# UoB-HPC/stdpar-nbody

Hardware: AMD Instinct MI355X
Metric: body-steps/sec + %FP64 peak, 3D double all-pairs N=2^20 at 1/2/4/8 GPUs (higher is better)
Workload: dtype f64

## Files before the change

### stdpar-nbody_amd/csrc/all_pairs.hip

```cpp
#include "common.hpp"

#include <atomic>
#include <cstdlib>
#include <mutex>
#include <type_traits>
#include <vector>

namespace nbody {

constexpr int kBlock = 256;
constexpr int kWaves = kBlock / 64;

struct ap_config {
  int split = 0;
  int tpt   = 0;
  int path  = 0;
};
static std::atomic<uint32_t> g_ap_default{0};

static ap_config ap_config_of(const nbody_state* s) {
  const uint32_t t = s->tuning ? s->tuning : g_ap_default.load(std::memory_order_relaxed);
  ap_config c;
  c.split = int(t & 15u);
  c.tpt   = int((t >> 4) & 3u);
  c.path  = int((t >> 6) & 3u);
  return c;
}

template <typename T, int D, int R, int JS>
__global__ __launch_bounds__(kBlock) void all_pairs_force_kernel(const T* __restrict__ m, const T* __restrict__ x,
                                                                 T* __restrict__ a, T c, uint32_t sz, uint32_t first,
                                                                 uint32_t count, const k1_rule* __restrict__ rule) {
  [[maybe_unused]] constexpr T e2 = T(0);
#define K1_SOFT false
#include "k1_tile_body.inc"
#undef K1_SOFT
}
template <typename T, int D, int R, int JS>
__global__ __launch_bounds__(kBlock) void all_pairs_softened_kernel(const T* __restrict__ m, const T* __restrict__ x,
                                                                    T* __restrict__ a, T c, uint32_t sz, uint32_t first,
                                                                    uint32_t count, T e2) {
  const k1_rule* const rule = nullptr;
#define K1_SOFT true
#include "k1_tile_body.inc"
#undef K1_SOFT
}

template <typename T, int D>
__global__ __launch_bounds__(kBlock) void pack_sources_kernel(const T* __restrict__ m, const T* __restrict__ x,
                                                              src_rec<T, D>* __restrict__ out, uint32_t sz, uint32_t padded) {
  const uint32_t j = blockIdx.x * kBlock + threadIdx.x;
  if (j >= padded) return;
  src_rec<T, D> r;
#pragma unroll
  for (int k = 0; k < 3; ++k) r.p[k] = (k < D && j < sz) ? x[uint64_t(j) * D + (k < D ? k : 0)] : T(0);
  r.m    = j < sz ? m[j] : T(0);
  out[j] = r;
}

template <typename T>
struct k1_prepare_tail {
  uint32_t turn_words;
};
template <>
struct k1_prepare_tail<double> {
  uint32_t turn_words;
  uint32_t bpc;
  double* cbox;
  double* pbox;
};
template <typename T, int D, bool PACK, bool MOMENTS>
__global__ __launch_bounds__(kBlock) void k1_prepare_kernel(const T* __restrict__ m, const T* __restrict__ x, src_rec<T, D>* __restrict__ out,
                                                            cst_batch* __restrict__ cst, uint32_t sz, uint32_t padded, k1_rule* rule, double* partial,
                                                            uint32_t* turn, k1_prepare_tail<T> tail) {
  constexpr bool BOX        = PACK && MOMENTS && sizeof(T) == 8;
  const uint32_t turn_words = tail.turn_words;
  [[maybe_unused]] uint32_t bpc = 0;
  [[maybe_unused]] T *cbox = nullptr, *pbox = nullptr;
  if constexpr (BOX) bpc = tail.bpc, cbox = tail.cbox, pbox = tail.pbox;
  const uint32_t j = blockIdx.x * kBlock + threadIdx.x;
  T p[D];
#pragma unroll
  for (int k = 0; k < D; ++k) p[k] = j < sz ? x[uint64_t(j) * D + k] : T(0);
  if constexpr (PACK) {
    if (j < padded) {
      src_rec<T, D> r;
#pragma unroll
      for (int k = 0; k < 3; ++k) r.p[k] = k < D ? p[k < D ? k : 0] : T(0);
      r.m    = j < sz ? m[j] : T(0);
      out[j] = r;
      if constexpr (sizeof(T) == 8) {
        const src_cst<T> k  = src_cst<T>::of(r.m);
        cst[j / 2].m15[j % 2]   = k.m15;
        cst[j / 2].m1875[j % 2] = k.m1875;
      }
    }
  }
  __shared__ double red[2 * D][kWaves];
  __shared__ T bred[BOX ? 2 * D : 1][kWaves];
  __shared__ bool last_s;
  const int lane = threadIdx.x & 63, wave = threadIdx.x >> 6;
  if constexpr (MOMENTS) {
    double s1[D], s2[D];
#pragma unroll
    for (int k = 0; k < D; ++k) {
      const double d = j < sz ? double(p[k]) - double(x[k]) : 0.0;
      s1[k] = d;
      s2[k] = d * d;
    }
#pragma unroll
    for (int k = 0; k < D; ++k)
      for (int off = 32; off > 0; off >>= 1) {
        s1[k] += __shfl_xor(s1[k], off, 64);
        s2[k] += __shfl_xor(s2[k], off, 64);
      }
    if (lane == 0) {
#pragma unroll
      for (int k = 0; k < D; ++k) {
        red[k][wave]     = s1[k];
        red[D + k][wave] = s2[k];
      }
    }
    if constexpr (BOX) {
      if (bpc != 0) {
        bool finite = true;
#pragma unroll
        for (int k = 0; k < D; ++k) finite = finite && (p[k] - p[k]) == T(0);
        T lo[D], hi[D];
#pragma unroll
        for (int k = 0; k < D; ++k) {
          lo[k] = finite ? p[k] : -T(__builtin_inf());
          hi[k] = finite ? p[k] : T(__builtin_inf());
        }
#pragma unroll
        for (int k = 0; k < D; ++k)
          for (int off = 32; off > 0; off >>= 1) {
            lo[k] = __builtin_fmin(lo[k], __shfl_xor(lo[k], off, 64));
            hi[k] = __builtin_fmax(hi[k], __shfl_xor(hi[k], off, 64));
          }
        if (lane == 0) {
#pragma unroll
          for (int k = 0; k < D; ++k) {
            bred[k][wave]     = lo[k];
            bred[D + k][wave] = hi[k];
          }
        }
      }
    }
    __syncthreads();
    if (threadIdx.x < 2 * D) {
      double v = red[threadIdx.x][0];
      for (int w = 1; w < kWaves; ++w) v += red[threadIdx.x][w];
      __hip_atomic_store(partial + size_t(blockIdx.x) * (2 * D) + threadIdx.x, v, __ATOMIC_RELAXED, __HIP_MEMORY_SCOPE_AGENT);
    }
    if constexpr (BOX) {
      if (bpc != 0 && threadIdx.x >= 64 && threadIdx.x < 64 + 2 * D) {
        const int q = int(threadIdx.x) - 64;
        T v         = bred[q][0];
        for (int w = 1; w < kWaves; ++w) v = q < D ? __builtin_fmin(v, bred[q][w]) : __builtin_fmax(v, bred[q][w]);
        __hip_atomic_store(pbox + size_t(blockIdx.x) * (2 * D) + q, v, __ATOMIC_RELAXED, __HIP_MEMORY_SCOPE_AGENT);
      }
    }
  }
  __builtin_amdgcn_s_waitcnt(0);
  __syncthreads();
  if (threadIdx.x == 0) last_s = __hip_atomic_fetch_add(&rule->ticket, 1u, __ATOMIC_RELAXED, __HIP_MEMORY_SCOPE_AGENT) == gridDim.x - 1u;
  __syncthreads();
  if (!last_s) return;
  if constexpr (MOMENTS) {
    double acc = 0.0;
    constexpr int G = kBlock / (2 * D), U = 8;
    const int q = threadIdx.x % (2 * D), g = threadIdx.x / (2 * D);
    if (g < G) {
      for (uint32_t b0 = uint32_t(g); b0 < gridDim.x; b0 += G * U) {
        double v[U];
#pragma unroll
        for (int u = 0; u < U; ++u) {
          const uint32_t b = b0 + uint32_t(u) * G;
          v[u] = b < gridDim.x ? __hip_atomic_load(partial + size_t(b) * (2 * D) + q, __ATOMIC_RELAXED, __HIP_MEMORY_SCOPE_AGENT) : 0.0;
        }
#pragma unroll
        for (int u = 0; u < U; ++u) acc += v[u];
      }
    }
    __shared__ double fin[kBlock];
    fin[threadIdx.x] = g < G ? acc : 0.0;
    __syncthreads();
    if (threadIdx.x < 2 * D) {
      double tot = 0.0;
#pragma unroll 6
      for (int gg = 0; gg < G; ++gg) tot += fin[gg * (2 * D) + threadIdx.x];
      fin[threadIdx.x] = tot;
    }
    __syncthreads();
    if (threadIdx.x == 0) {
      double vol = 1.0;
#pragma unroll
      for (int k = 0; k < D; ++k) {
        const double mean = fin[k] / double(sz), var = fin[D + k] / double(sz) - mean * mean;
        vol *= var > 0.0 ? __builtin_sqrt(12.0 * var) : 0.0;
      }
      rule->volume = vol;
      rule->sparse = vol >= kFarMinVolume<D> ? 1u : 0u;
    }
  }
  if constexpr (BOX) {
    if (bpc != 0) {
      const uint32_t nchunks = (gridDim.x + bpc - 1) / bpc;
      const uint32_t sub     = threadIdx.x & 15u;
      for (uint32_t c0 = 0; c0 < nchunks; c0 += kBlock / 16) {
        const uint32_t c  = c0 + (threadIdx.x >> 4);
        const uint32_t b1 = c < nchunks ? min(gridDim.x, (c + 1u) * bpc) : 0u;
        T lo[D], hi[D];
#pragma unroll
        for (int k = 0; k < D; ++k) lo[k] = T(__builtin_inf()), hi[k] = -T(__builtin_inf());
        for (uint32_t b0 = c * bpc + sub; b0 < b1; b0 += 16u * 4u) {
          T v[4][2 * D];
#pragma unroll
          for (int u = 0; u < 4; ++u) {
            const uint32_t b = b0 + 16u * uint32_t(u);
#pragma unroll
            for (int q = 0; q < 2 * D; ++q)
              v[u][q] = b < b1 ? __hip_atomic_load(pbox + size_t(b) * (2 * D) + q, __ATOMIC_RELAXED, __HIP_MEMORY_SCOPE_AGENT)
                               : (q < D ? T(__builtin_inf()) : -T(__builtin_inf()));
          }
#pragma unroll
          for (int u = 0; u < 4; ++u)
#pragma unroll
            for (int k = 0; k < D; ++k) {
              lo[k] = __builtin_fmin(lo[k], v[u][k]);
              hi[k] = __builtin_fmax(hi[k], v[u][D + k]);
            }
        }
#pragma unroll
        for (int k = 0; k < D; ++k)
          for (int off = 8; off > 0; off >>= 1) {
            lo[k] = __builtin_fmin(lo[k], __shfl_xor(lo[k], off, 64));
            hi[k] = __builtin_fmax(hi[k], __shfl_xor(hi[k], off, 64));
          }
        if (c < nchunks && sub == 0) {
#pragma unroll
          for (int k = 0; k < D; ++k) {
            cbox[size_t(c) * (2 * D) + k]     = lo[k];
            cbox[size_t(c) * (2 * D) + D + k] = hi[k];
          }
        }
      }
    }
  }
  for (uint32_t w = threadIdx.x; w < turn_words; w += kBlock) turn[w] = 0u;
  if (threadIdx.x == 0) __hip_atomic_store(&rule->ticket, 0u, __ATOMIC_RELAXED, __HIP_MEMORY_SCOPE_AGENT);
}

template <int JS>
constexpr int kSgprWaves = JS > kWaves ? JS : kWaves;

constexpr uint32_t kTurnSpins  = 1u << 26;
constexpr uint32_t kTurnPoison = 0xffffffffu;
struct k1_status {
  uint32_t err, block, group, chunk;
  unsigned long long polls, waits;
};
struct k1_handoff {
  void* sums;
  uint32_t* turn;
  k1_status* status;
  uint32_t spins;
  uint32_t delay;
  uint32_t late;
};
constexpr size_t kBoxHeaderBytes = 64;
template <typename T>
struct k1_rule_arg {
  const k1_rule* rule;
};
template <>
struct k1_rule_arg<double> {
  const k1_rule* rule;
  const double* box;
};
template <typename T, int D, int R, int JS, int RULE = 0>
__global__ __launch_bounds__(64 * kSgprWaves<JS>) void all_pairs_force_sgpr_kernel(const src_rec<T, D>* __restrict__ packed,
                                                                                   const cst_batch* __restrict__ cst,
                                                                                   const T* __restrict__ x, T* a, T c, uint32_t sz,
                                                                                   uint32_t first, uint32_t count,
                                                                                   uint32_t tiles_per_chunk, k1_handoff h,
                                                                                   k1_rule_arg<T> ra) {
  [[maybe_unused]] constexpr T e2 = T(0);
  const k1_rule* __restrict__ const rule = ra.rule;
  [[maybe_unused]] const T* __restrict__ box = nullptr;
  if constexpr (sizeof(T) == 8) box = ra.box;
#define K1_SOFT false
#include "k1_sgpr_body.inc"
#undef K1_SOFT
}
template <typename T, int D, int R, int JS>
__global__ __launch_bounds__(64 * kSgprWaves<JS>) void all_pairs_softened_sgpr_kernel(const src_rec<T, D>* __restrict__ packed,
                                                                                      const cst_batch* __restrict__ cst,
                                                                                      const T* __restrict__ x, T* a, T c, uint32_t sz,
                                                                                      uint32_t first, uint32_t count,
                                                                                      uint32_t tiles_per_chunk, k1_handoff h, T e2) {
  constexpr int RULE = 0;
  const k1_rule* const rule = nullptr;
  [[maybe_unused]] const T* const box = nullptr;
#define K1_SOFT true
#include "k1_sgpr_body.inc"
#undef K1_SOFT
}

namespace {
struct scratch_buf {
  void* ptr  = nullptr;
  size_t cap = 0;
};
struct packed_slot {
  int device;
  hipStream_t stream;
  scratch_buf buf[8];
  std::vector<void*> retired;
  bool k1_dirty  = false;
  bool k1_failed = false;
};
std::mutex g_packed_mu;
std::vector<packed_slot> g_packed_slots;
}

int ap_scratch_get(hipStream_t st, int which, size_t bytes, void** out) {
  const int dev = stream_device(st);
  std::lock_guard<std::mutex> lock(g_packed_mu);
  packed_slot* slot = nullptr;
  for (auto& sl : g_packed_slots)
    if (sl.stream == st && sl.device == dev) slot = &sl;
  if (slot && slot->buf[which].cap >= bytes) {
    *out = slot->buf[which].ptr;
    return NBODY_OK;
  }
  hipStreamCaptureStatus cs = hipStreamCaptureStatusNone;
  if (st != nullptr) (void)hipStreamIsCapturing(st, &cs);
  if (cs != hipStreamCaptureStatusNone) {
    set_error("all-pairs: the scratch buffers of this stream must exist before a step is recorded "
              "(call nbody_all_pairs_force once outside nbody_graph_begin/end, or use a context from nbody_create)");
    return NBODY_ERR_STATE;
  }
  if (!slot) {
    g_packed_slots.push_back({dev, st, {}, {}});
    slot = &g_packed_slots.back();
  }
  void* fresh = nullptr;
  NB_HIP(hipMalloc(&fresh, bytes));
  if (which == 4 || which == 3 || which == 7) {
    if (hipError_t e = hipMemsetAsync(fresh, 0, bytes, st); e != hipSuccess) {
      (void)hipFree(fresh);
      return hip_fail(e, "hipMemsetAsync(K1 scratch)", __FILE__, __LINE__);
    }
  }
  if (slot->buf[which].ptr) slot->retired.push_back(slot->buf[which].ptr);
  slot->buf[which].ptr = fresh;
  slot->buf[which].cap = bytes;
  *out                 = fresh;
  return NBODY_OK;
}

void ap_scratch_release(hipStream_t st) {
  const int dev = stream_device(st);
  std::lock_guard<std::mutex> lock(g_packed_mu);
  for (size_t i = 0; i < g_packed_slots.size(); ++i) {
    if (g_packed_slots[i].stream == st && g_packed_slots[i].device == dev) {
      for (auto& b : g_packed_slots[i].buf) (void)hipFree(b.ptr);
      for (void* p : g_packed_slots[i].retired) (void)hipFree(p);
      g_packed_slots.erase(g_packed_slots.begin() + long(i));
      return;
    }
  }
}

struct k1_plan {
  bool scalar = false;
  int r = 1, js = 4;
  uint32_t chunks = 1, tiles_per_chunk = 0;
};

static int auto_split(uint32_t sz) { return sz >= 2048u ? 8 : 4; }

void ap_auto_chunks(uint32_t sz, uint32_t* chunks, uint32_t* tiles_per_chunk) {
  const uint32_t ntiles = (sz + kTileJ - 1) / kTileJ;
  uint32_t y = 16;
  while (y < 64 && uint64_t(y) * 65536u < sz) y *= 2;
  if (y > ntiles) y = ntiles ? ntiles : 1;
  uint32_t tpc = ntiles ? (ntiles + y - 1) / y : 1;
  *tiles_per_chunk = tpc;
  *chunks          = ntiles ? (ntiles + tpc - 1) / tpc : 1;
}

template <typename T>
static int plan_all_pairs(const nbody_state* s, k1_plan* out) {
  const ap_config cfg = ap_config_of(s);
  k1_plan p;
  p.js = cfg.split ? cfg.split : auto_split(s->sz);
  p.r  = cfg.tpt;
  const uint64_t waves_r1 = (uint64_t(s->count) + 63) / 64 * uint64_t(p.js);
  p.scalar                = p.js == 8 || cfg.path == 2 || (cfg.path == 0 && waves_r1 >= 4096);
  if (p.js == 8 && cfg.path == 1) {
    set_error("all-pairs: the LDS-tile form has at most 4 source slices; sz = %u uses 8 (nbody_all_pairs_configure(4, ...) to force 4)",
              s->sz);
    return NBODY_ERR_ARG;
  }
  p.tiles_per_chunk = (s->sz + kTileJ - 1) / kTileJ;
  if (p.scalar && cfg.split == 0 && p.js == 8) ap_auto_chunks(s->sz, &p.chunks, &p.tiles_per_chunk);
  if (const char* e = experiment_env("NBODY_K1_CHUNKS"); e && p.scalar) {
    const uint32_t ntiles = (s->sz + kTileJ - 1) / kTileJ;
    uint32_t y            = uint32_t(atoi(e));
    if (y >= 1 && y <= ntiles) {
      p.tiles_per_chunk = (ntiles + y - 1) / y;
      p.chunks          = (ntiles + p.tiles_per_chunk - 1) / p.tiles_per_chunk;
    }
  }
  if (p.r == 0) {
    const uint64_t blocks_r2 = (uint64_t(s->count) + 127) / 128 * p.chunks;
    if (p.scalar) p.r = (sizeof(T) == 8 && blocks_r2 >= 4096) ? 2 : 1;
    else p.r = blocks_r2 * uint64_t(p.js) >= 8192 ? 2 : 1;
  }
  *out = p;
  return NBODY_OK;
}

int ap_pack_sources(const nbody_state* s, hipStream_t st, void** packed_out) {
  const uint32_t padded = (s->sz + kTileJ - 1) / kTileJ * kTileJ;
  const size_t tsz      = s->dtype == NBODY_F32 ? 4 : 8;
  void* scratch         = nullptr;
  if (int r = ap_scratch_get(st, 0, 4 * tsz * size_t(padded), &scratch)) return r;
  int rc = dispatch(s->dtype, s->dim, [&](auto tg) {
    using T         = typename decltype(tg)::type;
    constexpr int D = decltype(tg)::dim;
    hipLaunchKernelGGL((pack_sources_kernel<T, D>), dim3((padded + kBlock - 1) / kBlock), dim3(kBlock), 0, st,
                       static_cast<const T*>(s->m), static_cast<const T*>(s->x), static_cast<src_rec<T, D>*>(scratch), s->sz, padded);
    NB_HIP(hipGetLastError());
    return int(NBODY_OK);
  });
  *packed_out = scratch;
  return rc;
}

static size_t ap_cst_bytes(size_t padded) { return sizeof(cst_batch) * (padded / 2); }

static size_t ap_rule_bytes(uint32_t sz, int dim) {
  const size_t padded = (size_t(sz) + kTileJ - 1) / kTileJ * kTileJ;
  return 32 + sizeof(double) * 2 * size_t(dim) * (padded / kBlock);
}

static size_t ap_box_bytes(uint32_t sz, int dim) {
  const size_t ntiles = (size_t(sz) + kTileJ - 1) / kTileJ;
  return kBoxHeaderBytes + sizeof(double) * 2 * size_t(dim) * (ntiles + ntiles * (kTileJ / kBlock));
}
static bool k1_box_wanted(uint32_t sz, uint32_t chunks) { return sz >= kFarMinBodies && chunks > 1; }

template <typename T, int D>
static int ap_prepare(const nbody_state* s, hipStream_t st, bool pack, src_rec<T, D>** packed_out, const cst_batch** cst_out,
                      const k1_rule** rule_out, uint32_t* turn, size_t turn_words, bool with_rule = true, uint32_t box_tpc = 0,
                      const T** box_out = nullptr) {
  const uint32_t padded = (s->sz + kTileJ - 1) / kTileJ * kTileJ;
  const bool moments    = with_rule && s->sz >= kFarMinBodies;
  void* scratch         = nullptr;
  void* consts          = nullptr;
  if (pack) {
    if (int r = ap_scratch_get(st, 0, 4 * sizeof(T) * size_t(padded), &scratch)) return r;
    if (sizeof(T) == 8)
      if (int r = ap_scratch_get(st, 6, ap_cst_bytes(padded), &consts)) return r;
  }
  void* q = nullptr;
  if (int r = ap_scratch_get(st, 3, ap_rule_bytes(s->sz, D), &q)) return r;
  auto* rule    = static_cast<k1_rule*>(q);
  auto* partial = reinterpret_cast<double*>(static_cast<char*>(q) + 32);
  auto* out     = static_cast<src_rec<T, D>*>(scratch);
  auto* cst     = static_cast<cst_batch*>(consts);
  T *cbox = nullptr, *pbox = nullptr;
  uint32_t bpc = 0;
  if (sizeof(T) == 8 && pack && moments && box_tpc != 0) {
    void* b = nullptr;
    if (int r = ap_scratch_get(st, 7, ap_box_bytes(s->sz, D), &b)) return r;
    cbox = reinterpret_cast<T*>(static_cast<char*>(b) + kBoxHeaderBytes);
    pbox = cbox + size_t(2 * D) * (padded / kTileJ);
    bpc  = box_tpc * (kTileJ / kBlock);
  }
  const dim3 grid(padded / kBlock), block(kBlock);
  const T *m = static_cast<const T*>(s->m), *x = static_cast<const T*>(s->x);
  const uint32_t words = uint32_t(turn_words);
  k1_prepare_tail<T> tail{};
  tail.turn_words = words;
  if constexpr (sizeof(T) == 8) tail.bpc = bpc, tail.cbox = cbox, tail.pbox = pbox;
  if (pack && moments) hipLaunchKernelGGL((k1_prepare_kernel<T, D, true, true>), grid, block, 0, st, m, x, out, cst, s->sz, padded, rule, partial, turn, tail);
  else if (pack) hipLaunchKernelGGL((k1_prepare_kernel<T, D, true, false>), grid, block, 0, st, m, x, out, cst, s->sz, padded, rule, partial, turn, tail);
  else if (moments) hipLaunchKernelGGL((k1_prepare_kernel<T, D, false, true>), grid, block, 0, st, m, x, out, cst, s->sz, padded, rule, partial, turn, tail);
  NB_HIP(hipGetLastError());
  if (box_out) *box_out = cbox;
  if (packed_out) *packed_out = out;
  if (cst_out) *cst_out = cst;
  *rule_out = moments ? rule : nullptr;
  return NBODY_OK;
}

constexpr uint32_t kCollectMaxBlocks = 2048;
static bool k1_collect(uint32_t target_blocks, uint32_t chunks) {
  uint32_t limit = kCollectMaxBlocks;
  if (const char* e = experiment_env("NBODY_K1_COLLECT_MAX")) limit = uint32_t(atoi(e));
  return chunks > 1 && uint64_t(target_blocks) * chunks <= limit;
}
template <typename T, int D, int R, int JS>
static size_t k1_collect_bytes(uint32_t target_blocks, uint32_t chunks) {
  constexpr int TG = kSgprWaves<JS> / JS;
  return sizeof(T) * size_t(chunks) * target_blocks * TG * R * D * 64;
}

template <int R, int JS>
static size_t sgpr_turn_words(uint32_t count) {
  constexpr int TG = kSgprWaves<JS> / JS, TB = TG * 64 * R;
  return size_t((count + TB - 1) / TB) * TG;
}

template <typename T, int D, int R, int JS, bool SOFT>
static int launch_all_pairs_sgpr(const nbody_state* s, const k1_plan& plan, hipStream_t st, T e2) {
  constexpr int TB = (kSgprWaves<JS> / JS) * 64 * R;
  uint32_t blocks  = (s->count + TB - 1) / TB;
  if (blocks == 0) return NBODY_OK;
  k1_handoff h{nullptr, nullptr, nullptr, kTurnSpins, 0u, 0u};
  if (plan.chunks > 1) {
    void* q = nullptr;
    if (int r = ap_scratch_get(st, 1, sizeof(uint32_t) * sgpr_turn_words<R, JS>(s->count), &q)) return r;
    h.turn = static_cast<uint32_t*>(q);
    if (k1_collect(blocks, plan.chunks)) {
      if (int r = ap_scratch_get(st, 5, k1_collect_bytes<T, D, R, JS>(blocks, plan.chunks), &q)) return r;
      h.sums = q;
    }
    if (int r = ap_scratch_get(st, 4, sizeof(k1_status), &q)) return r;
    h.status = static_cast<k1_status*>(q);
    if (const char* e = experiment_env("NBODY_K1_TURN_SPINS")) h.spins = uint32_t(strtoul(e, nullptr, 10));
    if (const char* e = experiment_env("NBODY_K1_HANDOFF_DELAY")) h.delay = uint32_t(strtoul(e, nullptr, 10));
    if (const char* e = experiment_env("NBODY_K1_HANDOFF_LATE")) h.late = uint32_t(strtoul(e, nullptr, 10));
    if (const char* e = experiment_env("NBODY_K1_NO_HANDOFF"); e && e[0] == '1') h.turn = nullptr, h.sums = nullptr;
    if (const char* e = experiment_env("NBODY_K1_COLLECT"); e && e[0] == '0') h.sums = nullptr;
  }
  src_rec<T, D>* packed = nullptr;
  const cst_batch* cst  = nullptr;
  const k1_rule* rule   = nullptr;
  const T* box          = nullptr;
  bool certify          = !SOFT && sizeof(T) == 8 && k1_box_wanted(s->sz, plan.chunks);
  if (const char* e = experiment_env("NBODY_K1_NO_CERT"); e && e[0] == '1') certify = false;
  if (int r = ap_prepare<T, D>(s, st, true, &packed, &cst, &rule, h.turn, h.turn ? sgpr_turn_words<R, JS>(s->count) : 0, !SOFT,
                               certify ? plan.tiles_per_chunk : 0u, &box))
    return r;
  if constexpr (SOFT) {
    hipLaunchKernelGGL((all_pairs_softened_sgpr_kernel<T, D, R, JS>), dim3(blocks, plan.chunks), dim3(64 * kSgprWaves<JS>), 0, st,
                       packed, cst, static_cast<const T*>(s->x), static_cast<T*>(s->a), static_cast<T>(s->c), s->sz, s->first, s->count,
                       plan.tiles_per_chunk, h, e2);
    NB_HIP(hipGetLastError());
    if (h.turn != nullptr && h.sums == nullptr) ap_status_mark(st);
    return NBODY_OK;
  }
  k1_rule_arg<T> ra{};
  ra.rule = rule;
  if constexpr (sizeof(T) == 8) ra.box = box;
#ifdef NBODY_EXPERIMENTS
  if (const char* e = getenv("NBODY_K1_RULE_FORCE"); e && JS == 8 && D == 3) {
    if (e[0] == '1')
      hipLaunchKernelGGL((all_pairs_force_sgpr_kernel<T, D, R, JS, 1>), dim3(blocks, plan.chunks), dim3(64 * kSgprWaves<JS>), 0, st,
                         packed, cst, static_cast<const T*>(s->x), static_cast<T*>(s->a), static_cast<T>(s->c), s->sz, s->first, s->count,
                         plan.tiles_per_chunk, h, ra);
    else
      hipLaunchKernelGGL((all_pairs_force_sgpr_kernel<T, D, R, JS, 2>), dim3(blocks, plan.chunks), dim3(64 * kSgprWaves<JS>), 0, st,
                         packed, cst, static_cast<const T*>(s->x), static_cast<T*>(s->a), static_cast<T>(s->c), s->sz, s->first, s->count,
                         plan.tiles_per_chunk, h, ra);
    NB_HIP(hipGetLastError());
    return NBODY_OK;
  }
#endif
  hipLaunchKernelGGL((all_pairs_force_sgpr_kernel<T, D, R, JS>), dim3(blocks, plan.chunks), dim3(64 * kSgprWaves<JS>), 0, st,
                     packed, cst, static_cast<const T*>(s->x), static_cast<T*>(s->a), static_cast<T>(s->c), s->sz, s->first, s->count,
                     plan.tiles_per_chunk, h, ra);
  NB_HIP(hipGetLastError());
  if (h.turn != nullptr && h.sums == nullptr) ap_status_mark(st);
  return NBODY_OK;
}

template <typename T, int D, int R, int JS, bool SOFT>
static int launch_all_pairs(const nbody_state* s, hipStream_t st, T e2) {
  constexpr int TB = (kWaves / JS) * 64 * R;
  uint32_t blocks  = (s->count + TB - 1) / TB;
  if (blocks == 0) return NBODY_OK;
  if constexpr (SOFT) {
    hipLaunchKernelGGL((all_pairs_softened_kernel<T, D, R, JS>), dim3(blocks), dim3(kBlock), 0, st, static_cast<const T*>(s->m),
                       static_cast<const T*>(s->x), static_cast<T*>(s->a), static_cast<T>(s->c), s->sz, s->first, s->count, e2);
    NB_HIP(hipGetLastError());
    return NBODY_OK;
  }
  const k1_rule* rule = nullptr;
  if (int r = ap_prepare<T, D>(s, st, false, nullptr, nullptr, &rule, nullptr, 0)) return r;
  hipLaunchKernelGGL((all_pairs_force_kernel<T, D, R, JS>), dim3(blocks), dim3(kBlock), 0, st, static_cast<const T*>(s->m),
                     static_cast<const T*>(s->x), static_cast<T*>(s->a), static_cast<T>(s->c), s->sz, s->first, s->count, rule);
  NB_HIP(hipGetLastError());
  return NBODY_OK;
}

template <typename F>
static bool with_k1_instance(const k1_plan& p, F&& fn) {
#define NB_CASE(RR, JJ)                                                                       \
  if (p.r == RR && p.js == JJ) {                                                              \
    fn(std::integral_constant<int, RR>{}, std::integral_constant<int, JJ>{});                 \
    return true;                                                                              \
  }
  NB_CASE(1, 1);
  NB_CASE(1, 2);
  NB_CASE(1, 4);
  NB_CASE(2, 1);
  NB_CASE(2, 2);
  NB_CASE(2, 4);
  if (p.scalar) {
    NB_CASE(1, 8);
    NB_CASE(2, 8);
  }
#undef NB_CASE
  return false;
}

template <typename T, int D, bool SOFT = false>
static int all_pairs_dispatch(const nbody_state* s, hipStream_t st, T e2 = T(0)) {
  k1_plan p;
  if (int rc = plan_all_pairs<T>(s, &p)) return rc;
  int rc = NBODY_OK;
  const bool found = with_k1_instance(p, [&](auto r, auto js) {
    constexpr int R = decltype(r)::value, JS = decltype(js)::value;
    rc = p.scalar ? launch_all_pairs_sgpr<T, D, R, JS, SOFT>(s, p, st, e2)
                  : (JS <= kWaves ? launch_all_pairs<T, D, R, (JS <= kWaves ? JS : 1), SOFT>(s, st, e2) : int(NBODY_ERR_ARG));
  });
  if (!found) {
    set_error("all-pairs: unsupported config split=%d targets_per_thread=%d", p.js, p.r);
    return NBODY_ERR_ARG;
  }
  return rc;
}

template <typename T, int D>
static int all_pairs_describe(const nbody_state* s, char* out, size_t len) {
  k1_plan p;
  if (int rc = plan_all_pairs<T>(s, &p)) return rc;
  const char* t = sizeof(T) == 8 ? "double" : "float";
  const char* pair = sizeof(T) == 4 ? (s->sz >= kFarMinBodies ? "rsq+rcp[m y^3 at r2 >= 4 if sparse]" : "rsq+rcp")
                                    : s->sz >= kFarMinBodies ? "far3m[-eps if sparse]/near3" : "far3m/near3";
  if (p.scalar) {
    bool collect = false;
    with_k1_instance(p, [&](auto r, auto js) {
      constexpr int TB = (kSgprWaves<decltype(js)::value> / decltype(js)::value) * 64 * decltype(r)::value;
      collect = k1_collect((s->count + TB - 1) / TB, p.chunks);
    });
    snprintf(out, len, "all_pairs_force_sgpr_kernel<%s,%d,R=%d,JS=%d> tile=%d chunks=%u%s pair=%s%s", t, D, p.r, p.js, kTileJ, p.chunks,
             p.chunks > 1 ? (collect ? "(summed in chunk order by the last to arrive)" : "(summed in turn into a)") : "", pair,
             sizeof(T) == 8 && k1_box_wanted(s->sz, p.chunks) ? " cert=box-gap>=3[if sparse: blocks proven far skip the r2 test]" : "");
  }
  else
    snprintf(out, len, "all_pairs_force_kernel<%s,%d,R=%d,JS=%d> tile=%d chunks=1 pair=%s", t, D, p.r, p.js, kTileJ, pair);
  return NBODY_OK;
}

int ap_scratch_reserve(hipStream_t st, const nbody_state* s) {
  void* q             = nullptr;
  const size_t tsz    = s->dtype == NBODY_F32 ? 4 : 8;
  const size_t padded = (size_t(s->sz) + 2 * kTileJ - 1) / (2 * kTileJ) * (2 * kTileJ);
  if (int r = ap_scratch_get(st, 0, 4 * tsz * padded, &q)) return r;
  if (s->dtype == NBODY_F64)
    if (int r = ap_scratch_get(st, 6, ap_cst_bytes(padded), &q)) return r;
  if (int r = ap_scratch_get(st, 3, ap_rule_bytes(s->sz, s->dim), &q)) return r;
  if (s->dtype == NBODY_F64 && s->sz >= kFarMinBodies)
    if (int r = ap_scratch_get(st, 7, ap_box_bytes(s->sz, s->dim), &q)) return r;
  return dispatch(s->dtype, s->dim, [&](auto tg) {
    using T = typename decltype(tg)::type;
    k1_plan p;
    if (int rc = plan_all_pairs<T>(s, &p)) return rc;
    if (!p.scalar || p.chunks <= 1) return int(NBODY_OK);
    size_t words = 0;
    with_k1_instance(p, [&](auto r, auto js) { words = sgpr_turn_words<decltype(r)::value, decltype(js)::value>(s->count); });
    if (!words) return int(NBODY_OK);
    if (int rc = ap_scratch_get(st, 1, sizeof(uint32_t) * words, &q)) return rc;
    size_t sums = 0;
    with_k1_instance(p, [&](auto r, auto js) {
      constexpr int RR = decltype(r)::value, JJ = decltype(js)::value;
      const uint32_t blocks = (s->count + (kSgprWaves<JJ> / JJ) * 64 * RR - 1) / ((kSgprWaves<JJ> / JJ) * 64 * RR);
      if (k1_collect(blocks, p.chunks)) sums = k1_collect_bytes<T, decltype(tg)::dim, RR, JJ>(blocks, p.chunks);
    });
    if (sums)
      if (int rc = ap_scratch_get(st, 5, sums, &q)) return rc;
    return ap_scratch_get(st, 4, sizeof(k1_status), &q);
  });
}

void ap_status_mark(hipStream_t st) {
  const int dev = stream_device(st);
  std::lock_guard<std::mutex> lock(g_packed_mu);
  for (auto& sl : g_packed_slots)
    if (sl.stream == st && sl.device == dev) sl.k1_dirty = true;
}

int ap_status_read(hipStream_t st, unsigned long long out[6], bool clear) {
  const int dev = stream_device(st);
  k1_status* dptr = nullptr;
  {
    std::lock_guard<std::mutex> lock(g_packed_mu);
    for (auto& sl : g_packed_slots)
      if (sl.stream == st && sl.device == dev && (out != nullptr || sl.k1_dirty || sl.k1_failed)) dptr = static_cast<k1_status*>(sl.buf[4].ptr);
  }
  k1_status h{};
  if (dptr) NB_HIP(hipMemcpyAsync(&h, dptr, sizeof h, hipMemcpyDeviceToHost, st));
  NB_HIP(hipStreamSynchronize(st));
  if (dptr && clear && (h.err || h.polls || h.waits)) {
    NB_HIP(hipMemsetAsync(dptr, 0, sizeof h, st));
    NB_HIP(hipStreamSynchronize(st));
  }
  if (out) {
    out[0] = h.err, out[1] = h.block, out[2] = h.group, out[3] = h.chunk;
    out[4] = h.polls, out[5] = h.waits;
  }
  if (dptr) {
    std::lock_guard<std::mutex> lock(g_packed_mu);
    for (auto& sl : g_packed_slots)
      if (sl.stream == st && sl.device == dev) sl.k1_dirty = false, sl.k1_failed = h.err != 0 && !clear;
  }
  if (h.err) {
    set_error("all-pairs: the chunk hand-off of target block %u (group %u) failed at source chunk %u: the block of chunk %u never passed "
              "the turn on within the poll budget (workgroups not started in index order?).  `a` of that launch is not valid (the "
              "group's rows are NaN).  The flag is sticky for this stream until nbody_all_pairs_status(stream, out, 1)",
              h.block, h.group, h.chunk, h.chunk - 1u);
    return NBODY_ERR_STATE;
  }
  return NBODY_OK;
}

template <typename T>
constexpr int kColTileJ = sizeof(T) == 4 ? 2048 : 1024;

template <typename T, int D>
__global__ __launch_bounds__(kBlock) void collapsed_reset_kernel(T* __restrict__ a, const T* __restrict__ ao, uint64_t n) {
  uint64_t e = uint64_t(blockIdx.x) * kBlock + threadIdx.x;
  if (e < n) a[e] = a[e] - ao[e];
}

template <int CTRL, int ROW_MASK>
__device__ __forceinline__ int dpp_i32(int v) {
  return __builtin_amdgcn_update_dpp(0, v, CTRL, ROW_MASK, 0xf, false);
}
template <int CTRL, int ROW_MASK = 0xf>
__device__ __forceinline__ float dpp_get(float v) {
  return __builtin_bit_cast(float, dpp_i32<CTRL, ROW_MASK>(__builtin_bit_cast(int, v)));
}
template <int CTRL, int ROW_MASK = 0xf>
__device__ __forceinline__ double dpp_get(double v) {
  const long long b = __builtin_bit_cast(long long, v);
  const int lo = dpp_i32<CTRL, ROW_MASK>(int(b)), hi = dpp_i32<CTRL, ROW_MASK>(int(b >> 32));
  return __builtin_bit_cast(double, (long long)(((unsigned long long)(unsigned)hi << 32) | (unsigned)lo));
}

template <typename T>
__device__ __forceinline__ T lane_bcast(T v, int src) {
  if constexpr (sizeof(T) == 4) {
    return __builtin_bit_cast(T, __builtin_amdgcn_readlane(__builtin_bit_cast(int, v), src));
  } else {
    long long b = __builtin_bit_cast(long long, v);
    int lo      = __builtin_amdgcn_readlane(int(b), src);
    int hi      = __builtin_amdgcn_readlane(int(b >> 32), src);
    return __builtin_bit_cast(T, (long long)(((unsigned long long)(unsigned)hi << 32) | (unsigned)lo));
  }
}

template <typename T>
__device__ __forceinline__ T xor_lane_add(T v, int mask) {
  return v + __shfl_xor(v, mask, 64);
}

template <typename T, int NT>
__device__ __forceinline__ T transpose_reduce(T (&p)[NT], int lane) {
  static_assert(NT == 16 || NT == 8, "groups of 16 (f32) or 8 (f64) targets");
  if constexpr (NT == 16) {
    const bool up = (lane & 8) != 0;
#pragma unroll
    for (int i = 0; i < 8; ++i) {
      const T send = up ? p[i] : p[i + 8], keep = up ? p[i + 8] : p[i];
      p[i]         = keep + dpp_get<0x140>(send);
    }
  }
  {
    const bool up = (lane & 4) != 0;
#pragma unroll
    for (int i = 0; i < 4; ++i) {
      const T send = up ? p[i] : p[i + 4], keep = up ? p[i + 4] : p[i];
      p[i]         = keep + dpp_get<0x141>(send);
    }
  }
  {
    const bool up = (lane & 2) != 0;
#pragma unroll
    for (int i = 0; i < 2; ++i) {
      const T send = up ? p[i] : p[i + 2], keep = up ? p[i + 2] : p[i];
      p[i]         = keep + dpp_get<0x4E>(send);
    }
  }
  {
    const bool up = (lane & 1) != 0;
    const T send  = up ? p[0] : p[1], keep = up ? p[1] : p[0];
    p[0]          = keep + dpp_get<0xB1>(send);
  }
  T v = p[0];
  if constexpr (NT == 8) v += dpp_get<0x128>(v);
  v = xor_lane_add(v, 16);
  v = xor_lane_add(v, 32);
  return v;
}

struct k2_carry {
  float dx, dy, dz, r2, y;
};
__device__ __forceinline__ k2_carry k2_pair_head(const src_rec<float, 3>& s, const float (&xg)[3]) {
  k2_carry n;
  asm volatile(
      "v_subrev_f32 %[dx], %[X], %[sx]\n\t"
      "v_subrev_f32 %[dy], %[Y], %[sy]\n\t"
      "v_subrev_f32 %[dz], %[Z], %[sz]\n\t"
      "v_fmaak_f32 %[r2], %[dx], %[dx], 0x2081cea\n\t"
      "v_fmac_f32 %[r2], %[dy], %[dy]\n\t"
      "v_fmac_f32 %[r2], %[dz], %[dz]\n\t"
      "v_rsq_f32 %[y], %[r2]\n\t"
      "s_nop 0"
      : [dx] "=&v"(n.dx), [dy] "=&v"(n.dy), [dz] "=&v"(n.dz), [r2] "=&v"(n.r2), [y] "=&v"(n.y)
      : [sx] "v"(s.p[0]), [sy] "v"(s.p[1]), [sz] "v"(s.p[2]), [X] "s"(xg[0]), [Y] "s"(xg[1]), [Z] "s"(xg[2]));
  return n;
}
__device__ __forceinline__ k2_carry k2_pair_step(const src_rec<float, 3>& s, const float (&xg)[3], float mp, const k2_carry& c,
                                                 float& ax, float& ay, float& az) {
  k2_carry n;
  float t;
  asm volatile(
      "v_mul_f32 %[t], %[r2p], %[yp]\n\t"
      "v_subrev_f32 %[dx], %[X], %[sx]\n\t"
      "v_fmaak_f32 %[t], %[r2p], %[t], 0x34000000\n\t"
      "v_subrev_f32 %[dy], %[Y], %[sy]\n\t"
      "v_subrev_f32 %[dz], %[Z], %[sz]\n\t"
      "v_rcp_f32 %[t], %[t]\n\t"
      "v_fmaak_f32 %[r2], %[dx], %[dx], 0x2081cea\n\t"
      "v_fmac_f32 %[r2], %[dy], %[dy]\n\t"
      "v_fmac_f32 %[r2], %[dz], %[dz]\n\t"
      "v_mul_f32 %[t], %[mp], %[t]\n\t"
      "v_rsq_f32 %[y], %[r2]\n\t"
      "v_fmac_f32 %[ax], %[t], %[dxp]\n\t"
      "v_fmac_f32 %[ay], %[t], %[dyp]\n\t"
      "v_fmac_f32 %[az], %[t], %[dzp]"
      : [dx] "=&v"(n.dx), [dy] "=&v"(n.dy), [dz] "=&v"(n.dz), [r2] "=&v"(n.r2), [y] "=&v"(n.y), [t] "=&v"(t), [ax] "+v"(ax),
        [ay] "+v"(ay), [az] "+v"(az)
      : [sx] "v"(s.p[0]), [sy] "v"(s.p[1]), [sz] "v"(s.p[2]), [X] "s"(xg[0]), [Y] "s"(xg[1]), [Z] "s"(xg[2]), [mp] "v"(mp),
        [r2p] "v"(c.r2), [yp] "v"(c.y), [dxp] "v"(c.dx), [dyp] "v"(c.dy), [dzp] "v"(c.dz));
  return n;
}
__device__ __forceinline__ void k2_pair_tail(float mp, const k2_carry& c, float& ax, float& ay, float& az) {
  float t;
  asm volatile(
      "v_mul_f32 %[t], %[r2p], %[yp]\n\t"
      "v_fmaak_f32 %[t], %[r2p], %[t], 0x34000000\n\t"
      "v_rcp_f32 %[t], %[t]\n\t"
      "s_nop 0\n\t"
      "v_mul_f32 %[t], %[mp], %[t]\n\t"
      "v_fmac_f32 %[ax], %[t], %[dxp]\n\t"
      "v_fmac_f32 %[ay], %[t], %[dyp]\n\t"
      "v_fmac_f32 %[az], %[t], %[dzp]"
      : [t] "=&v"(t), [ax] "+v"(ax), [ay] "+v"(ay), [az] "+v"(az)
      : [mp] "v"(mp), [r2p] "v"(c.r2), [yp] "v"(c.y), [dxp] "v"(c.dx), [dyp] "v"(c.dy), [dzp] "v"(c.dz));
}

template <typename T, int D, int NT, int KS, int NB>
__global__ __launch_bounds__(kBlock) void all_pairs_collapsed_kernel(const T* __restrict__ m, const T* __restrict__ x,
                                                                     T* __restrict__ a, T c, uint32_t sz,
                                                                     uint32_t tiles_per_block) {
  using rec_t = src_rec<T, D>;
  constexpr int TJ = kColTileJ<T>;
  constexpr int KJ = TJ / 64;
  __shared__ rec_t tile[TJ];

  const int lane = threadIdx.x & 63;
  const int wave = threadIdx.x >> 6;
  const pair_consts<T> pc;

  const uint32_t i0   = (blockIdx.x * kWaves + wave) * 64;
  const uint32_t imy  = i0 + lane;
  const bool ivalid   = imy < sz;
  T xt[D], mine[D];
#pragma unroll
  for (int k = 0; k < D; ++k) {
    xt[k]   = x[uint64_t(ivalid ? imy : 0u) * D + k];
    mine[k] = T(0);
  }
  const int ngroups = (i0 < sz) ? int((min(64u, sz - i0) + NT - 1) / NT) : 0;

  const uint32_t ntiles = (sz + TJ - 1) / TJ;
  const uint32_t t0     = blockIdx.y * tiles_per_block;
  const uint32_t t1     = min(ntiles, t0 + tiles_per_block);

  for (uint32_t t = t0; t < t1; ++t) {
    __syncthreads();
#pragma unroll
    for (int q = 0; q < TJ / kBlock; ++q) {
      uint32_t slot = q * kBlock + threadIdx.x;
      uint64_t j    = uint64_t(t) * TJ + slot;
      rec_t r;
      if (j < sz) {
#pragma unroll
        for (int k = 0; k < D; ++k) r.p[k] = x[j * D + k];
        r.m = m[j];
      } else {
#pragma unroll
        for (int k = 0; k < D; ++k) r.p[k] = T(0);
        r.m = T(0);
      }
      if (D == 2) r.p[2] = T(0);
      tile[slot] = r;
    }
    __syncthreads();

    constexpr int SUBS = KJ / KS;
    for (int g = 0; g < ngroups; ++g) {
      T xg[NT][D];
#pragma unroll
      for (int tt = 0; tt < NT; ++tt)
#pragma unroll
        for (int k = 0; k < D; ++k) xg[tt][k] = lane_bcast(xt[k], g * NT + tt);
      T part[D][NT];
      bool guarded = sizeof(T) == 4;
      for (int pass = 0; pass < 2; ++pass) {
#pragma unroll
        for (int k = 0; k < D; ++k)
#pragma unroll
          for (int tt = 0; tt < NT; ++tt) part[k][tt] = T(0);
        uint32_t lowest = 0xffffffffu;
#pragma unroll 1
        for (int sub = 0; sub < SUBS; ++sub) {
          rec_t src[KS];
#pragma unroll
          for (int q = 0; q < KS; ++q) src[q] = tile[(sub * KS + q) * 64 + lane];
          if constexpr (NB == 0) {
            static_assert(NB != 0 || (sizeof(T) == 4 && D == 3), "the hand-scheduled pair is float 3D");
            k2_carry cy = k2_pair_head(src[0], xg[0]);
#pragma unroll
            for (int p = 1; p < NT * KS; ++p) {
              const int tp = (p - 1) / KS;
              cy = k2_pair_step(src[p % KS], xg[p / KS], src[(p - 1) % KS].m, cy, part[0][tp], part[1][tp], part[2][tp]);
            }
            k2_pair_tail(src[KS - 1].m, cy, part[0][NT - 1], part[1][NT - 1], part[2][NT - 1]);
          } else
#pragma unroll
          for (int tt = 0; tt < NT; ++tt) {
            T pt[D];
#pragma unroll
            for (int k = 0; k < D; ++k) pt[k] = part[k][tt];
            if constexpr (sizeof(T) == 8) {
              if (guarded) {
#pragma unroll
                for (int q = 0; q < KS; q += NB) pair_accumulate_multi<T, D, NB>(pt, xg[tt], &src[q]);
              } else {
#pragma unroll
                for (int q = 0; q < KS; q += NB) pair_accumulate_far<D, NB>(pt, xg[tt], &src[q], lowest, pc.k15, pc.k1875);
              }
            } else {
#pragma unroll
              for (int q = 0; q < KS; q += NB) pair_accumulate_multi<T, D, NB>(pt, xg[tt], &src[q]);
            }
#pragma unroll
            for (int k = 0; k < D; ++k) part[k][tt] = pt[k];
          }
        }
        if (guarded || __builtin_amdgcn_ballot_w64(lowest < pair_math<double>::near_hi) == 0ull) break;
        guarded = true;
      }
// ... 415 lines not shown
```

Baseline: 1.791 million.

## Sort bodies by Morton key before force kernel to tighten far-field box certification

Adds a per-step spatial reordering path for large sparse double runs. Bodies get 30-bit Morton keys, are radix-sorted, and the packed source records and constants are gathered in that order while per-chunk bounding boxes are rebuilt from the sorted data. Accelerations are then scattered back to the original order. Sorting makes tile boxes compact, so more tile pairs can be proven far and skip the r2 test. The cost is extra sort, gather and scatter kernels and scratch memory every step, and spatially clustered inputs gain nothing when the rule is not sparse.

```diff
diff --git a/stdpar-nbody_amd/csrc/all_pairs.hip b/stdpar-nbody_amd/csrc/all_pairs.hip
--- a/stdpar-nbody_amd/csrc/all_pairs.hip
+++ b/stdpar-nbody_amd/csrc/all_pairs.hip
@@ -1,4 +1,6 @@
 #include "common.hpp"
+#include "k1_order_key.hpp"
+#include "radix_sort.hpp"
 
 #include <atomic>
 #include <cstdlib>
@@ -316,7 +318,7 @@
 struct packed_slot {
   int device;
   hipStream_t stream;
-  scratch_buf buf[8];
+  scratch_buf buf[9];
   std::vector<void*> retired;
   bool k1_dirty  = false;
   bool k1_failed = false;
@@ -454,6 +456,210 @@
 }
 static bool k1_box_wanted(uint32_t sz, uint32_t chunks) { return sz >= kFarMinBodies && chunks > 1; }
 
+constexpr double kOrderSafe = 1e150;
+__device__ __forceinline__ double k1_order_safe(double p, bool on) { return on && p > kOrderSafe ? kOrderSafe : (on && p < -kOrderSafe ? -kOrderSafe : p); }
+constexpr uint32_t kOrderMinBodies = 262144;
+static bool k1_order_wanted(uint32_t sz, uint32_t chunks) {
+  if (const char* e = experiment_env("NBODY_K1_NO_ORDER"); e && e[0] == '1') return false;
+  uint32_t least = kOrderMinBodies;
+  if (const char* e = experiment_env("NBODY_K1_ORDER_MIN")) least = uint32_t(strtoul(e, nullptr, 10));
+  return k1_box_wanted(sz, chunks) && sz >= least;
+}
+
+struct k1_order_layout {
+  size_t recs, cst, keys[2], idx[2], hist, xs, as, bytes;
+};
+static k1_order_layout k1_order_layout_of(uint32_t sz, uint32_t count, int dim) {
+  const size_t padded = (size_t(sz) + kTileJ - 1) / kTileJ * kTileJ;
+  size_t at           = 0;
+  auto take = [&](size_t bytes) {
+    const size_t here = at;
+    at += (bytes + 255) / 256 * 256;
+    return here;
+  };
+  k1_order_layout l;
+  l.recs = take(32 * padded);
+  l.cst  = take(ap_cst_bytes(padded));
+  for (int b = 0; b < 2; ++b) l.keys[b] = take(sizeof(uint64_t) * sz);
+  for (int b = 0; b < 2; ++b) l.idx[b] = take(sizeof(uint32_t) * sz);
+  const size_t words = radix_sort_scratch_words(sz) > radix_sort_scratch_words(count) ? radix_sort_scratch_words(sz) : radix_sort_scratch_words(count);
+  l.hist  = take(sizeof(uint32_t) * words);
+  l.xs    = take(sizeof(double) * size_t(dim) * count);
+  l.as    = take(sizeof(double) * size_t(dim) * count);
+  l.bytes = at;
+  return l;
+}
+
+template <int D>
+__global__ __launch_bounds__(kBlock) void k1_order_key_kernel(const double* __restrict__ x, uint32_t first, uint32_t n,
+                                                              const k1_rule* __restrict__ rule, uint64_t* __restrict__ keys) {
+  const uint32_t i = blockIdx.x * kBlock + threadIdx.x;
+  if (i >= n) return;
+  double p[D];
+#pragma unroll
+  for (int k = 0; k < D; ++k) p[k] = x[(uint64_t(first) + i) * D + k];
+  keys[i] = rule->sparse ? k1_order_key<D>(p) : 0ull;
+}
+
+template <int D>
+__global__ __launch_bounds__(kBlock) void k1_order_gather_kernel(const src_rec<double, D>* __restrict__ in, const cst_batch* __restrict__ cin,
+                                                                 const uint32_t* __restrict__ perm, src_rec<double, D>* __restrict__ out,
+                                                                 cst_batch* __restrict__ cout, uint32_t sz, double* __restrict__ pbox,
+                                                                 double* __restrict__ xs, const k1_rule* __restrict__ rule) {
+  const uint32_t j   = blockIdx.x * kBlock + threadIdx.x;
+  const uint32_t src = j < sz ? perm[j] : j;
+  const bool safe    = rule->sparse != 0u;
+  src_rec<double, D> r = in[src];
+#pragma unroll
+  for (int k = 0; k < D; ++k) r.p[k] = k1_order_safe(r.p[k], safe);
+  out[j] = r;
+  cout[j / 2].m15[j % 2]     = cin[src / 2].m15[src % 2];
+  cout[j / 2].m1875[j % 2]   = cin[src / 2].m1875[src % 2];
+  if (xs != nullptr && j < sz) {
+#pragma unroll
+    for (int k = 0; k < D; ++k) xs[uint64_t(j) * D + k] = r.p[k];
+  }
+  bool finite = true;
+#pragma unroll
+  for (int k = 0; k < D; ++k) finite = finite && (r.p[k] - r.p[k]) == 0.0;
+  double lo[D], hi[D];
+#pragma unroll
+  for (int k = 0; k < D; ++k) {
+    lo[k] = finite ? r.p[k] : -__builtin_inf();
+    hi[k] = finite ? r.p[k] : __builtin_inf();
+  }
+#pragma unroll
+  for (int k = 0; k < D; ++k)
+    for (int off = 32; off > 0; off >>= 1) {
+      lo[k] = __builtin_fmin(lo[k], __shfl_xor(lo[k], off, 64));
+      hi[k] = __builtin_fmax(hi[k], __shfl_xor(hi[k], off, 64));
+    }
+  __shared__ double bred[2 * D][kWaves];
+  const int lane = threadIdx.x & 63, wave = threadIdx.x >> 6;
+  if (lane == 0) {
+#pragma unroll
+    for (int k = 0; k < D; ++k) {
+      bred[k][wave]     = lo[k];
+      bred[D + k][wave] = hi[k];
+    }
+  }
+  __syncthreads();
+  if (threadIdx.x < 2 * D) {
+    const int q = int(threadIdx.x);
+    double v    = bred[q][0];
+    for (int w = 1; w < kWaves; ++w) v = q < D ? __builtin_fmin(v, bred[q][w]) : __builtin_fmax(v, bred[q][w]);
+    pbox[size_t(blockIdx.x) * (2 * D) + q] = v;
+  }
+}
+
+template <int D>
+__global__ __launch_bounds__(kBlock) void k1_order_box_kernel(const double* __restrict__ pbox, uint32_t nblk, uint32_t bpc, double* __restrict__ cbox) {
+  const uint32_t b0 = blockIdx.x * bpc, b1 = min(nblk, b0 + bpc);
+  double lo[D], hi[D];
+#pragma unroll
+  for (int k = 0; k < D; ++k) lo[k] = __builtin_inf(), hi[k] = -__builtin_inf();
+  for (uint32_t b = b0 + threadIdx.x; b < b1; b += kBlock) {
+#pragma unroll
+    for (int k = 0; k < D; ++k) {
+      lo[k] = __builtin_fmin(lo[k], pbox[size_t(b) * (2 * D) + k]);
+      hi[k] = __builtin_fmax(hi[k], pbox[size_t(b) * (2 * D) + D + k]);
+    }
+  }
+#pragma unroll
+  for (int k = 0; k < D; ++k)
+    for (int off = 32; off > 0; off >>= 1) {
+      lo[k] = __builtin_fmin(lo[k], __shfl_xor(lo[k], off, 64));
+      hi[k] = __builtin_fmax(hi[k], __shfl_xor(hi[k], off, 64));
+    }
+  __shared__ double bred[2 * D][kWaves];
+  const int lane = threadIdx.x & 63, wave = threadIdx.x >> 6;
+  if (lane == 0) {
+#pragma unroll
+    for (int k = 0; k < D; ++k) {
+      bred[k][wave]     = lo[k];
+      bred[D + k][wave] = hi[k];
+    }
+  }
+  __syncthreads();
+  if (threadIdx.x < 2 * D) {
+    const int q = int(threadIdx.x);
+    double v    = bred[q][0];
+    for (int w = 1; w < kWaves; ++w) v = q < D ? __builtin_fmin(v, bred[q][w]) : __builtin_fmax(v, bred[q][w]);
+    cbox[size_t(blockIdx.x) * (2 * D) + q] = v;
+  }
+}
+
+template <int D>
+__global__ __launch_bounds__(kBlock) void k1_order_targets_kernel(const double* __restrict__ x, uint32_t first, uint32_t count,
+                                                                  const uint32_t* __restrict__ perm, double* __restrict__ xs,
+                                                                  const k1_rule* __restrict__ rule) {
+  const uint32_t k = blockIdx.x * kBlock + threadIdx.x;
+  if (k >= count) return;
+  const uint64_t i = uint64_t(first) + perm[k];
+  const bool safe  = rule->sparse != 0u;
+#pragma unroll
+  for (int d = 0; d < D; ++d) xs[uint64_t(k) * D + d] = k1_order_safe(x[i * D + d], safe);
+}
+
+template <int D>
+__global__ __launch_bounds__(kBlock) void k1_order_scatter_kernel(const uint64_t* __restrict__ as, uint32_t count, const uint32_t* __restrict__ perm,
+                                                                  uint64_t* __restrict__ a) {
+  const uint32_t k = blockIdx.x * kBlock + threadIdx.x;
+  if (k >= count) return;
+  const uint64_t i = perm[k];
+#pragma unroll
+  for (int d = 0; d < D; ++d) a[i * D + d] = as[uint64_t(k) * D + d];
+}
+
+template <int D>
+struct k1_ordered {
+  src_rec<double, D>* packed;
+  const cst_batch* cst;
+  const double* box;
+  const double* xs;
+  double* as;
+  const uint32_t* tperm;
+};
+
+template <int D>
+static int k1_order_queue(const nbody_state* s, hipStream_t st, const src_rec<double, D>* packed, const cst_batch* cst, const k1_rule* rule,
+                          uint32_t tpc, k1_ordered<D>* out) {
+  const uint32_t padded = (s->sz + kTileJ - 1) / kTileJ * kTileJ, nblk = padded / kBlock, bpc = tpc * (kTileJ / kBlock);
+  const k1_order_layout l = k1_order_layout_of(s->sz, s->count, D);
+  void *w = nullptr, *b = nullptr;
+  if (int r = ap_scratch_get(st, 8, l.bytes, &w)) return r;
+  if (int r = ap_scratch_get(st, 7, ap_box_bytes(s->sz, D), &b)) return r;
+  char* base = static_cast<char*>(w);
+  uint64_t* keys[2] = {reinterpret_cast<uint64_t*>(base + l.keys[0]), reinterpret_cast<uint64_t*>(base + l.keys[1])};
+  uint32_t* idx[2]  = {reinterpret_cast<uint32_t*>(base + l.idx[0]), reinterpret_cast<uint32_t*>(base + l.idx[1])};
+  uint32_t* hist    = reinterpret_cast<uint32_t*>(base + l.hist);
+  auto* recs        = reinterpret_cast<src_rec<double, D>*>(base + l.recs);
+  auto* csts        = reinterpret_cast<cst_batch*>(base + l.cst);
+  double* xs        = reinterpret_cast<double*>(base + l.xs);
+  double* cbox      = reinterpret_cast<double*>(static_cast<char*>(b) + kBoxHeaderBytes);
+  double* pbox      = cbox + size_t(2 * D) * (padded / kTileJ);
+  const double* x   = static_cast<const double*>(s->x);
+  const bool whole  = s->first == 0 && s->count == s->sz;
+  int fin           = 0;
+  hipLaunchKernelGGL((k1_order_key_kernel<D>), dim3((s->sz + kBlock - 1) / kBlock), dim3(kBlock), 0, st, x, 0u, s->sz, rule, keys[0]);
+  NB_HIP(hipGetLastError());
+  if (int r = radix_sort_pairs(keys, idx, s->sz, kOrderKeyBits, hist, st, &fin)) return r;
+  hipLaunchKernelGGL((k1_order_gather_kernel<D>), dim3(nblk), dim3(kBlock), 0, st, packed, cst, idx[fin], recs, csts, s->sz, pbox,
+                     whole ? xs : static_cast<double*>(nullptr), rule);
+  NB_HIP(hipGetLastError());
+  hipLaunchKernelGGL((k1_order_box_kernel<D>), dim3((nblk + bpc - 1) / bpc), dim3(kBlock), 0, st, pbox, nblk, bpc, cbox);
+  NB_HIP(hipGetLastError());
+  if (!whole) {
+    hipLaunchKernelGGL((k1_order_key_kernel<D>), dim3((s->count + kBlock - 1) / kBlock), dim3(kBlock), 0, st, x, s->first, s->count, rule, keys[0]);
+    NB_HIP(hipGetLastError());
+    if (int r = radix_sort_pairs(keys, idx, s->count, kOrderKeyBits, hist, st, &fin)) return r;
+    hipLaunchKernelGGL((k1_order_targets_kernel<D>), dim3((s->count + kBlock - 1) / kBlock), dim3(kBlock), 0, st, x, s->first, s->count, idx[fin], xs, rule);
+    NB_HIP(hipGetLastError());
+  }
+  *out = {recs, csts, cbox, xs, reinterpret_cast<double*>(base + l.as), idx[fin]};
+  return NBODY_OK;
+}
+
 template <typename T, int D>
 static int ap_prepare(const nbody_state* s, hipStream_t st, bool pack, src_rec<T, D>** packed_out, const cst_batch** cst_out,
                       const k1_rule** rule_out, uint32_t* turn, size_t turn_words, bool with_rule = true, uint32_t box_tpc = 0,
@@ -545,8 +751,9 @@
   const T* box          = nullptr;
   bool certify          = !SOFT && sizeof(T) == 8 && k1_box_wanted(s->sz, plan.chunks);
   if (const char* e = experiment_env("NBODY_K1_NO_CERT"); e && e[0] == '1') certify = false;
+  [[maybe_unused]] const bool ordered = certify && plan.chunks > 1 && k1_order_wanted(s->sz, plan.chunks);
   if (int r = ap_prepare<T, D>(s, st, true, &packed, &cst, &rule, h.turn, h.turn ? sgpr_turn_words<R, JS>(s->count) : 0, !SOFT,
-                               certify ? plan.tiles_per_chunk : 0u, &box))
+                               certify && !ordered ? plan.tiles_per_chunk : 0u, &box))
     return r;
   if constexpr (SOFT) {
     hipLaunchKernelGGL((all_pairs_softened_sgpr_kernel<T, D, R, JS>), dim3(blocks, plan.chunks), dim3(64 * kSgprWaves<JS>), 0, st,
@@ -573,6 +780,21 @@
     return NBODY_OK;
   }
 #endif
+  if constexpr (sizeof(T) == 8) {
+    if (ordered) {
+      k1_ordered<D> o{};
+      if (int r = k1_order_queue<D>(s, st, packed, cst, rule, plan.tiles_per_chunk, &o)) return r;
+      ra.box = o.box;
+      hipLaunchKernelGGL((all_pairs_force_sgpr_kernel<T, D, R, JS>), dim3(blocks, plan.chunks), dim3(64 * kSgprWaves<JS>), 0, st,
+                         o.packed, o.cst, o.xs, o.as, static_cast<T>(s->c), s->sz, 0u, s->count, plan.tiles_per_chunk, h, ra);
+      NB_HIP(hipGetLastError());
+      hipLaunchKernelGGL((k1_order_scatter_kernel<D>), dim3((s->count + kBlock - 1) / kBlock), dim3(kBlock), 0, st,
+                         reinterpret_cast<const uint64_t*>(o.as), s->count, o.tperm, static_cast<uint64_t*>(s->a));
+      NB_HIP(hipGetLastError());
+      if (h.turn != nullptr && h.sums == nullptr) ap_status_mark(st);
+      return NBODY_OK;
+    }
+  }
   hipLaunchKernelGGL((all_pairs_force_sgpr_kernel<T, D, R, JS>), dim3(blocks, plan.chunks), dim3(64 * kSgprWaves<JS>), 0, st,
                      packed, cst, static_cast<const T*>(s->x), static_cast<T*>(s->a), static_cast<T>(s->c), s->sz, s->first, s->count,
                      plan.tiles_per_chunk, h, ra);
@@ -653,7 +875,10 @@
     });
     snprintf(out, len, "all_pairs_force_sgpr_kernel<%s,%d,R=%d,JS=%d> tile=%d chunks=%u%s pair=%s%s", t, D, p.r, p.js, kTileJ, p.chunks,
              p.chunks > 1 ? (collect ? "(summed in chunk order by the last to arrive)" : "(summed in turn into a)") : "", pair,
-             sizeof(T) == 8 && k1_box_wanted(s->sz, p.chunks) ? " cert=box-gap>=3[if sparse: blocks proven far skip the r2 test]" : "");
+             sizeof(T) == 8 && k1_box_wanted(s->sz, p.chunks)
+                 ? (k1_order_wanted(s->sz, p.chunks) ? " cert=box-gap>=3[if sparse: blocks proven far skip the r2 test] order=morton30[if sparse]"
+                                                    : " cert=box-gap>=3[if sparse: blocks proven far skip the r2 test]")
+                 : "");
   }
   else
     snprintf(out, len, "all_pairs_force_kernel<%s,%d,R=%d,JS=%d> tile=%d chunks=1 pair=%s", t, D, p.r, p.js, kTileJ, pair);
@@ -670,6 +895,12 @@
   if (int r = ap_scratch_get(st, 3, ap_rule_bytes(s->sz, s->dim), &q)) return r;
   if (s->dtype == NBODY_F64 && s->sz >= kFarMinBodies)
     if (int r = ap_scratch_get(st, 7, ap_box_bytes(s->sz, s->dim), &q)) return r;
+  if (s->dtype == NBODY_F64) {
+    k1_plan p;
+    if (int rc = plan_all_pairs<double>(s, &p)) return rc;
+    if (p.scalar && k1_order_wanted(s->sz, p.chunks))
+      if (int r = ap_scratch_get(st, 8, k1_order_layout_of(s->sz, s->count, s->dim).bytes, &q)) return r;
+  }
   return dispatch(s->dtype, s->dim, [&](auto tg) {
     using T = typename decltype(tg)::type;
     k1_plan p;
diff --git a/stdpar-nbody_amd/csrc/k1_order_key.hpp b/stdpar-nbody_amd/csrc/k1_order_key.hpp
--- /dev/null
+++ b/stdpar-nbody_amd/csrc/k1_order_key.hpp
@@ -0,0 +1,39 @@
+#pragma once
+#include <cstdint>
+
+#if defined(__HIPCC__) || defined(__CUDACC__)
+#define NB_KEY_FN __host__ __device__ inline
+#else
+#define NB_KEY_FN inline
+#endif
+
+namespace nbody {
+
+constexpr int kOrderKeyBits    = 30;
+constexpr int kOrderAxisBits   = 10;
+constexpr double kOrderCell    = 1.0;
+constexpr double kOrderHalf    = 512.0;
+
+NB_KEY_FN uint32_t k1_order_cell(double x) {
+  if (!(x >= -kOrderHalf)) return 0u;
+  if (x >= kOrderHalf) return 1023u;
+  return uint32_t(int32_t(__builtin_floor(x / kOrderCell)) + int32_t(kOrderHalf));
+}
+
+NB_KEY_FN uint32_t k1_order_spread(uint32_t q) {
+  q &= 0x3ffu;
+  q = (q | (q << 16)) & 0x030000ffu;
+  q = (q | (q << 8)) & 0x0300f00fu;
+  q = (q | (q << 4)) & 0x030c30c3u;
+  q = (q | (q << 2)) & 0x09249249u;
+  return q;
+}
+
+template <int D>
+NB_KEY_FN uint64_t k1_order_key(const double* p) {
+  uint32_t key = 0;
+  for (int k = 0; k < D; ++k) key |= k1_order_spread(k1_order_cell(p[k])) << k;
+  return uint64_t(key);
+}
+
+}
```

New measurement: 1.859 million (median of 6 runs). 1.04x the previous value.
